# robotics-upo/social_force_window_planner

Measured on AMD Instinct MI355X. Metric: scored trajectories/sec (v x w samples x steps) @ N pedestrians; cmd_vel match, higher is better.
Workload: dtype f64

## Files before the change

include/sfw_hip.h:

```cpp
#ifndef SFW_HIP_H_
#define SFW_HIP_H_

#include <stdint.h>

#ifdef __cplusplus
extern "C" {
#endif

#define SFW_ABI_VERSION 2

typedef enum sfw_status {
  SFW_OK = 0,
  SFW_ERR_INVALID_ARG = -1,
  SFW_ERR_NO_DEVICE = -2,
  SFW_ERR_HIP = -3,
  SFW_ERR_STATE = -4,
  SFW_ERR_UNSUPPORTED = -5
} sfw_status;

#define SFW_COST_INVALID (-1.0)
#define SFW_COST_SKIPPED (-2.0)

#define SFW_ROBOT_ID_NONE INT32_MIN

// ... 109 lines not shown
int sfw_score_samples(sfw_handle h, const sfw_robot_state *rs, const double *vx, const double *vy,
                      const double *vtheta, int32_t n, const sfw_goal_args *args, double *costs_out,
                      sfw_best *best_out);

#define SFW_SEQ_MAX_KNOTS 64
int sfw_sequences_stage(sfw_handle h, const sfw_robot_state *rs, const double *vx, const double *vy,
                        const double *vtheta, int32_t n, int32_t K, const int32_t *knot_step,
                        const sfw_goal_args *args, int64_t index_base);
int sfw_score_sequences(sfw_handle h, const sfw_robot_state *rs, const double *vx, const double *vy,
                        const double *vtheta, int32_t n, int32_t K, const int32_t *knot_step,
                        const sfw_goal_args *args, double *costs_out, sfw_best *best_out);

#define SFW_PERTURB_KEEP_NOMINAL 1
#define SFW_PERTURB_NO_VY        2
#define SFW_PERTURB_KEEP_NORMALS 4
typedef struct sfw_perturb {
  uint64_t seed;
  const double *nominal;
  double sigma[3];
  double lo[3], hi[3];
  int32_t flags, reserved;
} sfw_perturb;
int sfw_sequences_perturb_stage(sfw_handle h, const sfw_robot_state *rs, const sfw_perturb *p, int32_t n, int32_t K,
                                const int32_t *knot_step, const sfw_goal_args *args, int64_t index_base);
int sfw_score_perturbed(sfw_handle h, const sfw_robot_state *rs, const sfw_perturb *p, int32_t n, int32_t K,
                        const int32_t *knot_step, const sfw_goal_args *args, double *costs_out, sfw_best *best_out);
int sfw_sequences_knots(sfw_handle h, int64_t first, int64_t count, double *vx_out, double *vy_out, double *vtheta_out);
int sfw_sequences_normals(sfw_handle h, int64_t first, int64_t count, double *z_out);

#define SFW_ORG_NONE 0
#define SFW_ORG_REGISTER_1 1
#define SFW_ORG_REGISTER_2 2
#define SFW_ORG_FLAT 3
typedef struct sfw_plan_info {
  int32_t split_step;
  int32_t levels;
  int32_t chunks;
  int32_t organisation;
  int64_t classes;
  int64_t class_steps;
  int64_t samples;
  int64_t flat_samples;
  int64_t one_launch;
  int64_t rest_noise_unreproduced;
} sfw_plan_info;
int sfw_grid_plan_info(sfw_handle h, sfw_plan_info *out);
int sfw_plan_shared_prefix(const double *linvels, int32_t nv,
                           const double *angvels, int32_t nw, double vx0,
                           double vtheta0, double acc_x, double acc_theta,
                           double sim_time, int32_t num_steps,
                           int32_t n_agents, int32_t *level_ends,
                           int64_t *level_classes, int32_t cap,
                           int32_t *n_levels);
int sfw_plan_axis_classes(const double *targets, int32_t n, double v0, double a_max, double dt, int32_t max_p,
                          int32_t form, int32_t *counts, int32_t *classes, int32_t *n_levels, int32_t *closed_form);
int sfw_plan_row_blocks(const double *linvels, int32_t nv, const double *angvels, int32_t nw, double vx0,
                        double vtheta0, double acc_x, double acc_theta, double sim_time, int32_t num_steps,
                        int32_t n_agents, int32_t R, int32_t *row0);
#define SFW_K2_AUTO (-1)
#define SFW_K2_REGISTER 0
#define SFW_K2_FLAT 1
int sfw_set_k2_form(sfw_handle h, int32_t form);
int sfw_set_timing(sfw_handle h, int32_t enabled);
int sfw_last_launch_ms(sfw_handle h, int32_t which, float *ms_out);
int sfw_last_clock_ghz(sfw_handle h, double *ghz_out);
int sfw_grid_points(sfw_handle h, int64_t index, double *points_xyth,
                    int32_t points_cap, int32_t *n_points);
int sfw_grid_points_batch(sfw_handle h, int64_t first, int64_t count, double *points_xyth, int32_t *n_points);
int sfw_set_points_capture(sfw_handle h, int32_t enabled);
int sfw_set_footprint_clearance(sfw_handle h, int32_t on);
int sfw_footprint_clearance_info(sfw_handle h, int32_t *built, int32_t *half_width);
int sfw_footprint_clearance_map(sfw_handle h, uint8_t *out, uint64_t cells);
void *sfw_stream(sfw_handle h);

#define SFW_TERM_VEL 0
#define SFW_TERM_DISTANCE 1
#define SFW_TERM_ANGLE 2
#define SFW_TERM_COSTMAP 3
#define SFW_TERM_SOCIAL 4
#define SFW_N_TERMS 5
#define SFW_RESCORE_MAX_K 1024
typedef struct sfw_weights {
  double vel, distance, angle, costmap, social;
} sfw_weights;
int sfw_set_terms_capture(sfw_handle h, int32_t enabled);
int sfw_grid_rescore(sfw_handle h, const sfw_weights *w, int32_t K, sfw_best *best_out, double *costs_out);
int sfw_grid_terms(sfw_handle h, int64_t first, int64_t count, double *terms_out);

#define SFW_BLEND_MAX_L 16
typedef struct sfw_blend_stat {
  double lambda;
  double j_min;
  double eta;
  double sum_w2;
  int64_t n_valid;
  int64_t index_min;
} sfw_blend_stat;
int sfw_grid_blend(sfw_handle h, const double *lambda, int32_t L, const double *bias,
                   sfw_blend_stat *stat_out, double *u_out, double *weights_out);

int sfw_sequences_control_cost(sfw_handle h, double gamma, double *bias_out);
int sfw_grid_blend_control(sfw_handle h, const double *lambda, int32_t L, double gamma, const double *bias,
                           sfw_blend_stat *stat_out, double *u_out, double *weights_out);

#define SFW_MPPI_MAX_ITER 32
typedef struct sfw_mppi {
// ... 158 lines not shown
```

social_force_window_planner_amd/_abi.py:

```python
import ctypes as C

SFW_OK = 0
SFW_ERR_INVALID_ARG = -1
SFW_ERR_NO_DEVICE = -2
SFW_ERR_HIP = -3
SFW_ERR_STATE = -4
SFW_ERR_UNSUPPORTED = -5

SFW_COST_INVALID = -1.0
SFW_COST_SKIPPED = -2.0

SFW_PRECISION_F64 = 0
SFW_PRECISION_F32 = 1
SFW_PRECISION_F64_STRICT = 2

SFW_K2_AUTO, SFW_K2_REGISTER, SFW_K2_FLAT = -1, 0, 1
SFW_ORG_NONE, SFW_ORG_REGISTER_1, SFW_ORG_REGISTER_2, SFW_ORG_FLAT = 0, 1, 2, 3


class SfwParams(C.Structure):
    _fields_ = [
        ("max_vel_x", C.c_double),
        ("sim_time", C.c_double),
        ("sim_granularity", C.c_double),
# ... 82 lines not shown

class SfwBest(C.Structure):
    _fields_ = [
        ("index", C.c_int64),
        ("cost", C.c_double),
        ("vx", C.c_double),
        ("vy", C.c_double),
        ("vtheta", C.c_double),
        ("n_valid", C.c_int64),
    ]

    def as_dict(self):
        return {n: getattr(self, n) for n, _ in self._fields_}


class SfwBestKey(C.Structure):
    _fields_ = [(n, C.c_double) for n in ("cost", "neg_linvel", "abs_angvel", "neg_index")]

    def as_tuple(self):
        return (self.cost, self.neg_linvel, self.abs_angvel, self.neg_index)


class SfwPlanInfo(C.Structure):
    _fields_ = [("split_step", C.c_int32), ("levels", C.c_int32), ("chunks", C.c_int32), ("organisation", C.c_int32),
                ("classes", C.c_int64), ("class_steps", C.c_int64), ("samples", C.c_int64), ("flat_samples", C.c_int64),
                ("one_launch", C.c_int64), ("rest_noise_unreproduced", C.c_int64)]

    def as_dict(self):
        return {"split_step": self.split_step, "levels": self.levels, "chunks": self.chunks, "classes": self.classes,
                "class_steps": self.class_steps, "samples": self.samples, "organisation": self.organisation,
                "flat_samples": self.flat_samples, "one_launch": self.one_launch,
                "rest_noise_unreproduced": self.rest_noise_unreproduced}


EXPORTED_SYMBOLS = (
    "sfw_params_default",
    "sfw_abi_version",
    "sfw_create",
    "sfw_destroy",
    "sfw_set_params",
    "sfw_last_error",
    "sfw_set_costmap",
    "sfw_set_footprint",
    "sfw_set_agents",
    "sfw_score_grid",
    "sfw_score_one",
    "sfw_grid_stage",
    "sfw_grid_launch",
    "sfw_grid_sync",
    "sfw_grid_fetch",
    "sfw_grid_costs_view",
    "sfw_grid_plan_info",
    "sfw_plan_shared_prefix",
    "sfw_plan_row_blocks",
    "sfw_plan_axis_classes",
    "sfw_set_k2_form",
    "sfw_set_timing",
    "sfw_last_launch_ms",
    "sfw_last_clock_ghz",
    "sfw_grid_points",
    "sfw_grid_points_batch",
    "sfw_set_points_capture",
    "sfw_stream",
    "sfw_multi_create",
    "sfw_multi_destroy",
    "sfw_multi_last_error",
    "sfw_multi_describe",
    "sfw_multi_ranks",
    "sfw_multi_rank_handle",
    "sfw_multi_set_params",
    "sfw_multi_set_costmap",
    "sfw_multi_set_footprint",
    "sfw_multi_set_agents",
    "sfw_multi_score_grid",
    "sfw_multi_rank_rows",
    "sfw_multi_last_us",
    "sfw_multi_grid_points",
    "sfw_batch_create",
    "sfw_batch_destroy",
    "sfw_batch_last_error",
    "sfw_batch_size",
    "sfw_batch_member",
    "sfw_batch_launch",
    "sfw_batch_fetch",
    "sfw_batch_score_grid",
    "sfw_batch_describe",
    "sfw_batch_last_us",
    "sfw_batch_set_list_fusion",
    "sfw_batch_get_list_fusion",
    "sfw_batch_score_samples",
    "sfw_batch_score_sequences",
    "sfw_batch_score_perturbed",
    "sfw_ensemble_set_list_fusion",
    "sfw_ensemble_get_list_fusion",
    "sfw_ensemble_batch_desc",
    "sfw_set_terms_capture",
    "sfw_grid_rescore",
    "sfw_grid_terms",
    "sfw_ensemble_create",
    "sfw_ensemble_destroy",
    "sfw_ensemble_last_error",
    "sfw_ensemble_size",
    "sfw_ensemble_member",
    "sfw_ensemble_set_params",
    "sfw_ensemble_set_costmap",
    "sfw_ensemble_set_footprint",
# ... 156 lines not shown
```

social_force_window_planner_amd/csrc/sfw_capi.hip:

```cpp

#include "sfw_device.h"

#include <dlfcn.h>
#include <link.h>

#include <algorithm>
#include <chrono>
#include <cmath>
#include <condition_variable>
#include <functional>
#include <mutex>
#include <thread>
#include <cstdio>
#include <cstdlib>
#include <cstring>
#include <limits>
#include <new>
#include <string>
#include <vector>

namespace {

template <typename T> struct dev_buf {
  T *p = nullptr;
// ... 605 lines not shown
      while (l > 0 && t_at(l - 1) > d) --l;
      lo.push_back(static_cast<int32_t>(l));
      hi.push_back(static_cast<int32_t>(h));
      int32_t classes = (l > 0 ? 1 : 0) + (h < cnt ? 1 : 0);
      if (h > l) classes += run[h - 1] - run[l] + 1;
      n.push_back(classes);
      if (static_cast<size_t>(classes) == cnt) break;
    }
    c.assign(n.size(), std::vector<int32_t>());
    return true;
  }
  void write_level(size_t lv) const {
    const size_t cnt = targets.size();
    const size_t l = static_cast<size_t>(lo[lv]), h = static_cast<size_t>(hi[lv]);
    std::vector<int32_t> &out = c[lv];
    out.resize(cnt);
    const int32_t below = l > 0 ? 1 : 0;
    const int32_t mid = h > l ? run[h - 1] - run[l] + 1 : 0;
    for (size_t k = 0; k < cnt; ++k) {
      int32_t id;
      if (k < l) id = 0;
      else if (k < h) id = below + (run[k] - run[l]);
      else id = below + mid;
      out[static_cast<size_t>(order[k])] = id;
    }
  }
};
bool plan_fast_allowed() {
  static const bool on = [] {
    const char *e = std::getenv("SFW_PLAN_GENERIC");
    return !(e && e[0] == '1');
  }();
  return on;
}
axis_classes classes_of_axis(const std::vector<double> &targets, double v0, double a_max, double dt, int max_p,
                             bool allow_fast = plan_fast_allowed()) {
  axis_classes a;
  a.targets = targets;
  a.v0 = v0;
  a.a_max = a_max;
  a.dt = dt;
  a.max_p = max_p;
  a.build(allow_fast);
  return a;
}
int prefix_max_p(int S) { return std::min(S - 1, 48); }

struct prefix_classes {
  axis_classes rows, own_cols;
  const axis_classes *cols = nullptr;
  int max_p = 0;
  int32_t n_rows_at(int p) const { return rows.n[std::min<size_t>(static_cast<size_t>(p), rows.n.size()) - 1]; }
  int32_t n_cols_at(int p) const { return cols->n[std::min<size_t>(static_cast<size_t>(p), cols->n.size()) - 1]; }
};

void classes_of_grid(prefix_classes &pc, const std::vector<double> &lin, const std::vector<double> &ang, double vx0,
                     double vth0, double acc_x, double acc_theta, double dt, int S, const axis_classes *shared_cols = nullptr) {
  pc.max_p = prefix_max_p(S);
  pc.rows = classes_of_axis(lin, vx0, acc_x, dt, pc.max_p);
  if (shared_cols && shared_cols->made_for(ang, vth0, acc_theta, dt, pc.max_p)) {
    pc.cols = shared_cols;
  } else {
    pc.own_cols = classes_of_axis(ang, vth0, acc_theta, dt, pc.max_p);
    pc.cols = &pc.own_cols;
  }
}

std::vector<int> choose_levels(const prefix_classes &pc, int64_t T, int S, double samples_per_wave, int cus) {
  std::vector<int> steps;
  const double full = step_cost(static_cast<double>(T), samples_per_wave, cus);
  const int last_p = std::min<int>(pc.max_p, static_cast<int>(std::max(pc.rows.n.size(), pc.cols->n.size())));
  std::vector<double> best(static_cast<size_t>(last_p) + 1, 0.0);
  std::vector<int> from(static_cast<size_t>(last_p) + 1, 0);
  double best_total = S * full;
  int best_end = 0;
  for (int p = 1; p <= last_p; ++p) {
    const double c = step_cost(static_cast<double>(pc.n_rows_at(p)) * pc.n_cols_at(p), samples_per_wave, cus);
    const double launch_cost = c < 1.0 ? 0.4 : 1.0;
    best[p] = 1e300;
    for (int q = 0; q < p; ++q) {
      const double v = best[q] + (p - q) * c + launch_cost;
      if (v < best[p]) { best[p] = v; from[p] = q; }
    }
    const double total = best[p] + (S - p) * full;
    if (total < best_total) { best_total = total; best_end = p; }
  }
  if (best_total > 0.97 * S * full) return steps;
  for (int p = best_end; p > 0; p = from[p]) steps.push_back(p);
  std::reverse(steps.begin(), steps.end());
  return steps;
}

void plan_row_blocks(const std::vector<double> &lin, const std::vector<double> &ang, double vx0, double vth0, double acc_x,
                     double acc_theta, double dt, int S, int A, int R, int form, int cus, std::vector<int32_t> &row0) {
  const int64_t nv = static_cast<int64_t>(lin.size()), nw = static_cast<int64_t>(ang.size());
  row0.assign(static_cast<size_t>(R) + 1, 0);
  for (int r = 0; r <= R; ++r) row0[static_cast<size_t>(r)] = static_cast<int32_t>((static_cast<int64_t>(r) * nv) / R);
  if (R <= 1 || A < 2 || S < 2 || (nv / R) * nw < 4096) return;
  prefix_classes pc;
  classes_of_grid(pc, lin, ang, vx0, vth0, acc_x, acc_theta, dt, S);
  const std::vector<int> steps = choose_levels(pc, nv * nw, S, static_cast<double>(sfw_samples_per_wave(A, (nv / R) * nw, form, cus)), cus);
  if (steps.empty()) return;
  std::vector<double> w(static_cast<size_t>(nv), static_cast<double>(nw) * (S - steps.back()));
  int prev = 0;
  for (int p : steps) {
    const std::vector<int32_t> &rc = pc.rows.level(p);
    const double per_class = static_cast<double>(pc.n_cols_at(p)) * (p - prev);
    for (int64_t i = 0; i < nv; ++i)
      if (i == 0 || rc[static_cast<size_t>(i)] != rc[static_cast<size_t>(i - 1)]) w[static_cast<size_t>(i)] += per_class;
    prev = p;
  }
  double total = 0.0;
  for (double v : w) total += v;
  double run = 0.0;
  int r = 1;
  for (int64_t i = 0; i < nv && r < R; ++i) {
    run += w[static_cast<size_t>(i)];
    while (r < R && run >= total * r / R) row0[static_cast<size_t>(r++)] = static_cast<int32_t>(i + 1);
  }
  for (; r < R; ++r) row0[static_cast<size_t>(r)] = static_cast<int32_t>(nv);
}

int plan_prefix(sfw_handle h, int64_t chunk, int S) {
  h->st.prefix_steps.clear();
  h->st.prefix_chunks.clear();
  h->st.cls_ints.clear();
  h->st.cls_max = 0;
  h->st.prefix_class_steps = h->st.prefix_last_classes = 0;
  const int64_t T = static_cast<int64_t>(h->st.nv) * h->st.nw;
  const bool forced = !h->cfg.prefix_env.empty();
  if (h->st.list) return SFW_OK;
  if ((forced && h->cfg.prefix_env[0] == 0) || h->st.A < 2 || S < 2 || h->st.vy_samp != 0.0) return SFW_OK;
  if (!forced && T < 4096) return SFW_OK;
  const int64_t rows_per_chunk = chunk / h->st.nw;
  if (rows_per_chunk < 1) return SFW_OK;
  prefix_classes pc;
  classes_of_grid(pc, h->st.lin, h->st.ang, h->st.rs.vx, h->st.rs.vtheta, h->st.ga.acc_x, h->st.ga.acc_theta, h->live.params.sim_time / S, S,
                  static_cast<const axis_classes *>(h->shared_cols));
  const axis_classes &rc = pc.rows, &cc = *pc.cols;
  const std::vector<int32_t> &nr = pc.rows.n, &nc = pc.cols->n;
  auto level = [](const axis_classes &c, int p) -> const std::vector<int32_t> & { return c.level(p); };
  auto count_at = [](const std::vector<int32_t> &n, int p) { return n[std::min<size_t>(static_cast<size_t>(p), n.size()) - 1]; };
  std::vector<int> steps;
  if (forced) {
    for (int p : h->cfg.prefix_env)
      if (p >= 1 && p <= pc.max_p) steps.push_back(p);
  } else {
    steps = choose_levels(pc, T, S, static_cast<double>(sfw_samples_per_wave(h->st.A, std::min<int64_t>(T, rows_per_chunk * h->st.nw), h->live.k2_form, h->cfg.n_cu)), h->cfg.n_cu);
  }
  if (steps.empty()) return SFW_OK;
  const size_t n_lv = steps.size();

  std::vector<int32_t> ints;
  ints.swap(h->st.cls_ints);
  ints.clear();
  ints.reserve(static_cast<size_t>(2 * n_lv + 2) * static_cast<size_t>(h->st.nv + h->st.nw));
  auto append = [&](const std::vector<int32_t> &v) {
    const size_t o = ints.size();
    ints.insert(ints.end(), v.begin(), v.end());
    return o;
  };
  std::vector<int32_t> ids;
  auto relabel = [&ids](const std::vector<int32_t> &cls, int64_t i0, int64_t i1, std::vector<int32_t> &local,
                        std::vector<int32_t> &rep) {
    ids.assign(cls.size(), -1);
    local.clear();
    rep.clear();
    local.reserve(static_cast<size_t>(i1 - i0));
    rep.reserve(static_cast<size_t>(i1 - i0));
    for (int64_t i = i0; i < i1; ++i) {
      int32_t &id = ids[static_cast<size_t>(cls[static_cast<size_t>(i)])];
      if (id < 0) {
        id = static_cast<int32_t>(rep.size());
        rep.push_back(static_cast<int32_t>(i - i0));
      }
      local.push_back(id);
    }
  };
  struct axis_level { std::vector<int32_t> local, rep, src; };
  auto axis_levels = [&](const axis_classes &cls, int64_t i0, int64_t i1) {
    std::vector<axis_level> out(n_lv);
    for (size_t l = 0; l < n_lv; ++l) {
      relabel(level(cls, steps[l]), i0, i1, out[l].local, out[l].rep);
      if (l > 0) {
        out[l].src.reserve(out[l].rep.size());
        for (int32_t r : out[l].rep) out[l].src.push_back(out[l - 1].local[static_cast<size_t>(r)]);
      }
    }
    return out;
  };
  const std::vector<axis_level> cols = axis_levels(cc, 0, h->st.nw);
  std::vector<size_t> o_col_rep(n_lv), o_col_src(n_lv);
  for (size_t l = 0; l < n_lv; ++l) {
    o_col_rep[l] = append(cols[l].rep);
    o_col_src[l] = append(cols[l].src);
  }
  h->st.prefix_o_col_cls = append(cols[n_lv - 1].local);
  int64_t max_cls = 0;
  for (int64_t r0 = 0; r0 < h->st.nv; r0 += rows_per_chunk) {
    const int64_t r1 = std::min<int64_t>(h->st.nv, r0 + rows_per_chunk);
    const std::vector<axis_level> rows = axis_levels(rc, r0, r1);
    chunk_plan cp;
    for (size_t l = 0; l < n_lv; ++l) {
      level_tables t;
      t.n_row = static_cast<int32_t>(rows[l].rep.size());
      t.n_col = static_cast<int32_t>(cols[l].rep.size());
      t.o_row_rep = append(rows[l].rep);
      t.o_row_src = append(rows[l].src);
      t.o_col_rep = o_col_rep[l];
      t.o_col_src = o_col_src[l];
      cp.lv.push_back(t);
      const int64_t n = static_cast<int64_t>(t.n_row) * t.n_col;
      max_cls = std::max(max_cls, n);
      h->st.prefix_class_steps += n * (steps[l] - (l ? steps[l - 1] : 0));
      if (l + 1 == n_lv) h->st.prefix_last_classes += n;
    }
    cp.o_row_cls = append(rows[n_lv - 1].local);
    h->st.prefix_chunks.push_back(cp);
  }
  h->st.cls_ints.swap(ints);
  h->st.cls_max = max_cls;
  h->st.cls_two = n_lv > 1;
  if (std::getenv("SFW_DEBUG_PLAN")) {
    std::fprintf(stderr, "[sfw] shared prefix, %d x %d samples, S=%d, %zu chunk(s):", h->st.nv, h->st.nw, S, h->st.prefix_chunks.size());
    for (size_t l = 0; l < n_lv; ++l)
      std::fprintf(stderr, " [%d,%d) %d x %d;", l ? steps[l - 1] : 0, steps[l], count_at(nr, steps[l]), count_at(nc, steps[l]));
    std::fprintf(stderr, " [%d,%d) samples\n", steps.back(), S);
  }
  h->st.prefix_steps = steps;
  h->st.prefix_S = S;
  h->st.prefix_chunk = rows_per_chunk * h->st.nw;
  return SFW_OK;
}

void rest_forces(const sfw_params &p, const std::vector<std::pair<int32_t, int32_t>> &pairs, const double *pos, const double *vel,
                 int A, double *out) {
  for (int i = 0; i < 2 * A; ++i) out[i] = 0.0;
  for (const auto &pr : pairs) {
    const int i = pr.first, j = pr.second;
    const double dx = pos[2 * j] - pos[2 * i], dy = pos[2 * j + 1] - pos[2 * i + 1];
    const double dn = std::sqrt(dx * dx + dy * dy);
    if (!(dn > 0.0)) continue;
    const double ux = dx / dn, uy = dy / dn;
    const double wx = vel[2 * i] - vel[2 * j], wy = vel[2 * i + 1] - vel[2 * j + 1];
    const double ix = p.sfm_lambda * wx + ux, iy = p.sfm_lambda * wy + uy;
    const double il = std::sqrt(ix * ix + iy * iy);
    if (!(il > 0.0)) continue;
    const double ex = ix / il, ey = iy / il;
    double theta = std::atan2(uy, ux) - std::atan2(ey, ex);
    while (theta <= -M_PI) theta += 2.0 * M_PI;
    while (theta > M_PI) theta -= 2.0 * M_PI;
    const double B = p.sfm_gamma * il;
    if (theta != 0.0) {
      const double sq = p.sfm_n * B * theta;
      const double fa = -(theta > 0.0 ? 1.0 : -1.0) * std::exp(-dn / B - sq * sq);
      out[2 * i] += p.sfm_force_factor_social * fa * -ey;
      out[2 * i + 1] += p.sfm_force_factor_social * fa * ex;
    }
  }
}

bool pinned_rest_table(const sfw_params &p, const sfw_robot_state &rs, const double *pos, const sfw_agent_const *cst, int A,
                       double *out) {
  bool any = false;
  for (int i = 1; i < A; ++i) any |= (cst[i].desired_velocity == 0.0);
  if (!any) return false;
  out[0] = rs.x;
  out[1] = rs.y;
  out[2] = out[3] = 0.0;
  for (int i = 0; i < A; ++i) out[4 + i] = 0.0;
  auto pair_at_rest = [&](double mx, double my, double ox, double oy, double &fx, double &fy, double &lx, double &ly) {
    fx = fy = lx = ly = 0.0;
    const double dx = ox - mx, dy = oy - my;
    const double dn = std::sqrt(dx * dx + dy * dy);
    if (!(dn > 0.0)) return;
    const double ux = dx / dn, uy = dy / dn;
    const double ix = p.sfm_lambda * 0.0 + ux, iy = p.sfm_lambda * 0.0 + uy;
    const double il = std::sqrt(ix * ix + iy * iy);
    if (!(il > 0.0)) return;
// ... 1609 lines not shown
  const size_t rows = 3 * static_cast<size_t>(h->st.nk), row = sizeof(double) * static_cast<size_t>(count);
  SFW_HIP(h, hipSetDevice(h->device));
  if (rows * row > h->pin_knots.cap) SFW_HIP(h, hipStreamSynchronize(h->stream));
  SFW_HIP(h, h->pin_knots.reserve(rows * row));
  SFW_HIP(h, hipMemcpy2DAsync(h->pin_knots.p, row, h->normals.p + first, sizeof(double) * static_cast<size_t>(n), row, rows,
                              hipMemcpyDeviceToHost, h->stream));
  SFW_HIP(h, wait_stream(h));
  std::memcpy(z_out, h->pin_knots.p, rows * row);
  return SFW_OK;
}

int sfw_score_one(sfw_handle h, const sfw_robot_state *rs, double vx_samp, double vy_samp, double vtheta_samp,
                  const sfw_goal_args *args, double *cost_out, double *points_xyth, int32_t points_cap,
                  int32_t *n_points) {
  if (!h) return SFW_ERR_INVALID_ARG;
  if (!cost_out) return fail(h, SFW_ERR_INVALID_ARG, "score_one: cost_out is NULL");
  if (int e = stage_one(h, rs, args, vx_samp, vy_samp, vtheta_samp)) return e;
  consume_stage consumed{h};
  const int S = num_steps_of(h->live.params);
  const size_t head = kOneHead, pts_bytes = sizeof(double) * 3 * static_cast<size_t>(S);
  sfw_launch L;
  fill_launch(h, L, 0, 1, 1);
  L.force_alive = (points_xyth && points_cap > 0) || n_points ? 1 : 0;
  {
    sfw_launch C = L;
    C.sel_out = nullptr;
    C.cycle_counter = nullptr;
    if (sfw_cycle_applies(C)) {
      if (head + pts_bytes > h->pin_one.cap) SFW_HIP(h, hipStreamSynchronize(h->stream));
      SFW_HIP(h, h->pin_one.reserve(head + pts_bytes));
      score_one_outputs_at(C, h->pin_one.p);
      arena_by_kernel(h, C);
      SFW_HIP(h, launch_cycle_of(C, h->stream));
      SFW_HIP(h, arena_fetched(h));
      SFW_HIP(h, wait_stream(h));
      score_one_unpack(h->pin_one.p, cost_out, points_xyth, points_cap, n_points);
      return SFW_OK;
    }
    if (int e = flush_arena(h)) return e;
  }
  SFW_HIP(h, h->one_out.reserve(head + pts_bytes));
  score_one_outputs_at(L, h->one_out.p);
  SFW_HIP(h, sfw_launch_rollout(L, h->stream));
  SFW_HIP(h, launch_social_of(L, h->stream));
  if (L.path_on) SFW_HIP(h, sfw_launch_path_add(L.costs, L.path_p, h->st.path_weight, 0, 1, h->stream));
  const size_t fetch = head + ((points_xyth && points_cap > 0) ? pts_bytes : 0);
  SFW_HIP(h, h->pin_out.reserve(fetch));
  SFW_HIP(h, hipMemcpyAsync(h->pin_out.p, h->one_out.p, fetch, hipMemcpyDeviceToHost, h->stream));
  SFW_HIP(h, hipStreamSynchronize(h->stream));
  score_one_unpack(h->pin_out.p, cost_out, points_xyth, points_cap, n_points);
  return SFW_OK;
}

int sfw_plan_shared_prefix(const double *linvels, int32_t nv, const double *angvels, int32_t nw, double vx0, double vtheta0,
                           double acc_x, double acc_theta, double sim_time, int32_t num_steps, int32_t n_agents,
                           int32_t *level_ends, int64_t *level_classes, int32_t cap, int32_t *n_levels) {
  if (!linvels || !angvels || nv <= 0 || nw <= 0 || num_steps < 1 || !n_levels || cap < 0 ||
      (cap > 0 && (!level_ends || !level_classes)))
    return SFW_ERR_INVALID_ARG;
  *n_levels = 0;
  const int64_t T = static_cast<int64_t>(nv) * nw;
  if (n_agents < 2 || num_steps < 2 || T < 4096) return SFW_OK;
  const std::vector<double> lin(linvels, linvels + nv), ang(angvels, angvels + nw);
  prefix_classes pc;
  classes_of_grid(pc, lin, ang, vx0, vtheta0, acc_x, acc_theta, sim_time / num_steps, num_steps);
  const int cus = env_device_cus(SFW_DEFAULT_CUS);
  const std::vector<int> steps = choose_levels(pc, T, num_steps, static_cast<double>(sfw_samples_per_wave(n_agents, T, SFW_K2_AUTO, cus)), cus);
  *n_levels = static_cast<int32_t>(steps.size());
  for (size_t l = 0; l < steps.size() && l < static_cast<size_t>(cap); ++l) {
    level_ends[l] = steps[l];
    level_classes[l] = static_cast<int64_t>(pc.n_rows_at(steps[l])) * pc.n_cols_at(steps[l]);
  }
  return SFW_OK;
}

int sfw_plan_axis_classes(const double *targets, int32_t n, double v0, double a_max, double dt, int32_t max_p, int32_t form,
                          int32_t *counts, int32_t *classes, int32_t *n_levels, int32_t *closed_form) {
  if (!targets || n <= 0 || max_p < 1 || !counts || !n_levels || (form != 0 && form != 1)) return SFW_ERR_INVALID_ARG;
  if (!all_finite(targets, static_cast<size_t>(n)) || !std::isfinite(v0) || !std::isfinite(a_max) || !std::isfinite(dt))
    return SFW_ERR_INVALID_ARG;
  const axis_classes a = classes_of_axis(std::vector<double>(targets, targets + n), v0, a_max, dt, max_p, form == 0);
  *n_levels = static_cast<int32_t>(a.n.size());
  if (closed_form) *closed_form = a.fast ? 1 : 0;
  for (size_t l = 0; l < a.n.size(); ++l) {
    counts[l] = a.n[l];
    if (classes) std::memcpy(classes + l * static_cast<size_t>(n), a.level(static_cast<int>(l) + 1).data(), sizeof(int32_t) * static_cast<size_t>(n));
  }
  return SFW_OK;
}

int sfw_plan_row_blocks(const double *linvels, int32_t nv, const double *angvels, int32_t nw, double vx0, double vtheta0,
                        double acc_x, double acc_theta, double sim_time, int32_t num_steps, int32_t n_agents, int32_t R,
                        int32_t *row0) {
  if (!linvels || !angvels || nv <= 0 || nw <= 0 || num_steps < 1 || R < 1 || !row0) return SFW_ERR_INVALID_ARG;
  if (!all_finite(linvels, static_cast<size_t>(nv)) || !all_finite(angvels, static_cast<size_t>(nw))) return SFW_ERR_INVALID_ARG;
  const std::vector<double> lin(linvels, linvels + nv), ang(angvels, angvels + nw);
  std::vector<int32_t> cuts;
  plan_row_blocks(lin, ang, vx0, vtheta0, acc_x, acc_theta, sim_time / num_steps, num_steps, n_agents, R, SFW_K2_AUTO,
                  env_device_cus(SFW_DEFAULT_CUS), cuts);
  std::memcpy(row0, cuts.data(), sizeof(int32_t) * (static_cast<size_t>(R) + 1));
  return SFW_OK;
}

int sfw_grid_plan_info(sfw_handle h, sfw_plan_info *out) {
  if (!h || !out) return SFW_ERR_INVALID_ARG;
  if (!h->st.valid) return fail(h, SFW_ERR_STATE, "grid_plan_info before grid_stage");
  const int64_t T = static_cast<int64_t>(h->st.nv) * h->st.nw;
  out->split_step = h->st.prefix_steps.empty() ? 0 : h->st.prefix_steps.back();
  out->levels = static_cast<int32_t>(h->st.prefix_steps.size());
  out->samples = T;
  out->classes = h->st.prefix_last_classes;
  out->class_steps = h->st.prefix_class_steps;
  if (!h->st.prefix_steps.empty()) {
    out->chunks = static_cast<int32_t>(h->st.prefix_chunks.size());
  } else {
    int64_t chunk = h->st.table_chunk;
    if (chunk > T) chunk = T;
    out->chunks = chunk > 0 ? static_cast<int32_t>((T + chunk - 1) / chunk) : 0;
  }
  out->organisation = sfw_social_organisation(h->st.A, out->chunks > 0 ? (T + out->chunks - 1) / out->chunks : T, h->st.O, h->live.k2_form, h->cfg.n_cu);
  out->flat_samples = sfw_social_flat_items(h->st.A, h->st.O, h->st.NG, out->chunks > 0 ? (T + out->chunks - 1) / out->chunks : T, h->live.k2_form, h->cfg.n_cu);
  out->rest_noise_unreproduced = rest_noise_unreproduced(h) ? 1 : 0;
  out->one_launch = 0;
  if (out->chunks == 1 && h->st.prefix_steps.empty()) {
    sfw_launch L;
    fill_launch(h, L, 0, T, T);
// ... 1885 lines not shown
```

social_force_window_planner_amd/planner.py:

```python
from __future__ import annotations

import ctypes as C
import os
import subprocess

import numpy as np

from ._abi import (
    EXPORTED_SYMBOLS,
    SFW_ENSEMBLE_MAX,
    SFW_ENSEMBLE_MEAN,
    SFW_ERR_NO_DEVICE,
    SFW_OK,
    SfwAgent,
    SfwBatchDesc,
    SfwBest,
    SfwBestKey,
    SfwBlendStat,
    SFW_BLEND_MAX_L,
    SfwGoalArgs,
    SfwMppi,
    SFW_MPPI_MAX_ITER,
    SfwParams,
    SfwPerturb,
# ... 43 lines not shown
        L.sfw_params_default.argtypes = [C.POINTER(SfwParams)]
        L.sfw_params_default.restype = None
        L.sfw_abi_version.restype = C.c_int
        L.sfw_create.argtypes = [C.POINTER(SfwParams), C.c_int, C.POINTER(vp)]
        L.sfw_destroy.argtypes = [vp]
        L.sfw_set_params.argtypes = [vp, C.POINTER(SfwParams)]
        L.sfw_last_error.argtypes = [vp]
        L.sfw_last_error.restype = C.c_char_p
        L.sfw_set_costmap.argtypes = [vp, vp, C.c_uint32, C.c_uint32, C.c_double, C.c_double, C.c_double]
        L.sfw_set_footprint.argtypes = [vp, vp, C.c_int32]
        L.sfw_set_agents.argtypes = [vp, vp, C.c_int32, vp, C.c_int32]
        L.sfw_score_grid.argtypes = [vp, C.POINTER(SfwRobotState), vp, C.c_int32, vp, C.c_int32,
                                     C.POINTER(SfwGoalArgs), vp, C.POINTER(SfwBest)]
        L.sfw_score_one.argtypes = [vp, C.POINTER(SfwRobotState), C.c_double, C.c_double, C.c_double,
                                    C.POINTER(SfwGoalArgs), C.POINTER(C.c_double), vp, C.c_int32,
                                    C.POINTER(C.c_int32)]
        L.sfw_grid_stage.argtypes = [vp, C.POINTER(SfwRobotState), vp, C.c_int32, vp, C.c_int32,
                                     C.POINTER(SfwGoalArgs), C.c_int64]
        L.sfw_grid_launch.argtypes = [vp]
        L.sfw_grid_sync.argtypes = [vp]
        L.sfw_grid_fetch.argtypes = [vp, vp, C.POINTER(SfwBest), C.POINTER(SfwBestKey)]
        L.sfw_grid_plan_info.argtypes = [vp, C.POINTER(SfwPlanInfo)]
        L.sfw_set_k2_form.argtypes = [vp, C.c_int32]
        L.sfw_set_timing.argtypes = [vp, C.c_int32]
        L.sfw_last_launch_ms.argtypes = [vp, C.c_int32, C.POINTER(C.c_float)]
        L.sfw_last_clock_ghz.argtypes = [vp, C.POINTER(C.c_double)]
        L.sfw_grid_points.argtypes = [vp, C.c_int64, vp, C.c_int32, C.POINTER(C.c_int32)]
        L.sfw_grid_points_batch.argtypes = [vp, C.c_int64, C.c_int64, vp, vp]
        L.sfw_set_points_capture.argtypes = [vp, C.c_int32]
        L.sfw_stream.argtypes = [vp]
        L.sfw_stream.restype = vp
        L.sfw_multi_create.argtypes = [C.POINTER(SfwParams), C.POINTER(C.c_int), C.c_int32, C.c_int32, C.POINTER(vp)]
        L.sfw_multi_destroy.argtypes = [vp]
        L.sfw_multi_last_error.argtypes = [vp]
        L.sfw_multi_last_error.restype = C.c_char_p
        L.sfw_multi_ranks.argtypes = [vp]
        L.sfw_multi_ranks.restype = C.c_int32
        L.sfw_multi_rank_handle.argtypes = [vp, C.c_int32]
        L.sfw_multi_rank_handle.restype = vp
        L.sfw_multi_set_params.argtypes = [vp, C.POINTER(SfwParams)]
        L.sfw_multi_set_costmap.argtypes = [vp, vp, C.c_uint32, C.c_uint32, C.c_double, C.c_double, C.c_double]
        L.sfw_multi_set_footprint.argtypes = [vp, vp, C.c_int32]
        L.sfw_multi_set_agents.argtypes = [vp, vp, C.c_int32, vp, C.c_int32]
        L.sfw_multi_score_grid.argtypes = [vp, C.POINTER(SfwRobotState), vp, C.c_int32, vp, C.c_int32,
                                           C.POINTER(SfwGoalArgs), vp, C.POINTER(SfwBest)]
        L.sfw_multi_last_us.argtypes = [vp, C.c_int32, C.POINTER(C.c_double)]
        L.sfw_multi_rank_rows.argtypes = [vp, C.c_int32, C.POINTER(C.c_int32), C.POINTER(C.c_int32)]
        L.sfw_plan_row_blocks.argtypes = [vp, C.c_int32, vp, C.c_int32, C.c_double, C.c_double, C.c_double, C.c_double,
                                          C.c_double, C.c_int32, C.c_int32, C.c_int32, vp]
        L.sfw_grid_costs_view.argtypes = [vp]
        L.sfw_grid_costs_view.restype = C.c_void_p
        L.sfw_plan_shared_prefix.argtypes = [vp, C.c_int32, vp, C.c_int32, C.c_double, C.c_double, C.c_double, C.c_double,
                                             C.c_double, C.c_int32, C.c_int32, vp, vp, C.c_int32, C.POINTER(C.c_int32)]
        L.sfw_multi_grid_points.argtypes = [vp, C.c_int64, vp, C.c_int32, C.POINTER(C.c_int32)]
        L.sfw_batch_create.argtypes = [C.POINTER(SfwParams), C.c_int, C.c_int32, C.POINTER(vp)]
        L.sfw_batch_destroy.argtypes = [vp]
        L.sfw_batch_last_error.argtypes = [vp]
        L.sfw_batch_last_error.restype = C.c_char_p
        L.sfw_batch_size.argtypes = [vp]
        L.sfw_batch_size.restype = C.c_int32
        L.sfw_batch_member.argtypes = [vp, C.c_int32]
        L.sfw_batch_member.restype = vp
        L.sfw_batch_launch.argtypes = [vp]
        L.sfw_batch_fetch.argtypes = [vp, vp]
        L.sfw_batch_score_grid.argtypes = [vp, vp, vp, C.c_int32, vp, C.c_int32, vp, vp]
        L.sfw_batch_describe.argtypes = [vp, C.POINTER(SfwBatchDesc)]
        L.sfw_batch_last_us.argtypes = [vp, C.c_int32, C.POINTER(C.c_double)]
        L.sfw_set_terms_capture.argtypes = [vp, C.c_int32]
        L.sfw_grid_rescore.argtypes = [vp, C.POINTER(SfwWeights), C.c_int32, C.POINTER(SfwBest), vp]
        L.sfw_grid_terms.argtypes = [vp, C.c_int64, C.c_int64, vp]
        L.sfw_ensemble_create.argtypes = [C.POINTER(SfwParams), C.c_int, C.c_int32, C.POINTER(vp)]
        L.sfw_ensemble_destroy.argtypes = [vp]
        L.sfw_ensemble_last_error.argtypes = [vp]
        L.sfw_ensemble_last_error.restype = C.c_char_p
        L.sfw_ensemble_size.argtypes = [vp]
        L.sfw_ensemble_size.restype = C.c_int32
        L.sfw_ensemble_member.argtypes = [vp, C.c_int32]
        L.sfw_ensemble_member.restype = vp
        L.sfw_ensemble_set_params.argtypes = [vp, C.POINTER(SfwParams)]
        L.sfw_ensemble_set_costmap.argtypes = [vp, vp, C.c_uint32, C.c_uint32, C.c_double, C.c_double, C.c_double]
        L.sfw_ensemble_set_footprint.argtypes = [vp, vp, C.c_int32]
        L.sfw_ensemble_set_hypothesis.argtypes = [vp, C.c_int32, vp, C.c_int32, vp, C.c_int32]
        L.sfw_ensemble_score_grid.argtypes = [vp, C.POINTER(SfwRobotState), vp, C.c_int32, vp, C.c_int32,
                                              C.POINTER(SfwGoalArgs), C.c_int32, vp, vp, vp, C.POINTER(SfwBest)]
        L.sfw_ensemble_aggregate.argtypes = [vp, C.c_int32, vp, vp, vp, C.POINTER(SfwBest)]
        L.sfw_ensemble_last_us.argtypes = [vp, C.c_int32, C.POINTER(C.c_double)]
        L.sfw_samples_stage.argtypes = [vp, C.POINTER(SfwRobotState), vp, vp, vp, C.c_int32, C.POINTER(SfwGoalArgs), C.c_int64]
        L.sfw_score_samples.argtypes = [vp, C.POINTER(SfwRobotState), vp, vp, vp, C.c_int32, C.POINTER(SfwGoalArgs), vp,
                                        C.POINTER(SfwBest)]
        L.sfw_score_one_crowd.argtypes = [vp, C.POINTER(SfwRobotState), C.c_double, C.c_double, C.c_double,
                                          C.POINTER(SfwGoalArgs), C.POINTER(C.c_double), vp, vp, vp, C.c_int32, C.c_int32,
                                          C.POINTER(C.c_int32)]
        L.sfw_grid_crowd.argtypes = [vp, C.c_int64, C.POINTER(C.c_double), vp, vp, vp, C.c_int32, C.c_int32,
                                     C.POINTER(C.c_int32)]
        L.sfw_sequences_stage.argtypes = [vp, C.POINTER(SfwRobotState), vp, vp, vp, C.c_int32, C.c_int32, vp,
                                          C.POINTER(SfwGoalArgs), C.c_int64]
        L.sfw_score_sequences.argtypes = [vp, C.POINTER(SfwRobotState), vp, vp, vp, C.c_int32, C.c_int32, vp,
                                          C.POINTER(SfwGoalArgs), vp, C.POINTER(SfwBest)]
        L.sfw_grid_blend.argtypes = [vp, vp, C.c_int32, vp, C.POINTER(SfwBlendStat), vp, vp]
        L.sfw_sequences_perturb_stage.argtypes = [vp, C.POINTER(SfwRobotState), C.POINTER(SfwPerturb), C.c_int32, C.c_int32, vp,
                                                  C.POINTER(SfwGoalArgs), C.c_int64]
        L.sfw_score_perturbed.argtypes = [vp, C.POINTER(SfwRobotState), C.POINTER(SfwPerturb), C.c_int32, C.c_int32, vp,
                                          C.POINTER(SfwGoalArgs), vp, C.POINTER(SfwBest)]
        L.sfw_sequences_knots.argtypes = [vp, C.c_int64, C.c_int64, vp, vp, vp]
        L.sfw_sequences_normals.argtypes = [vp, C.c_int64, C.c_int64, vp]
        L.sfw_ensemble_score_sequences.argtypes = [vp, C.POINTER(SfwRobotState), vp, vp, vp, C.c_int32, C.c_int32, vp,
# ... 493 lines not shown
        if count is None:
            nv, nw = self._grid if self._grid is not None else (0, 0)
            count = max(nv * nw - first, 0)
        out = np.empty((count, SFW_N_TERMS), dtype=np.float64)
        self._check(lib().sfw_grid_terms(self._h, first, count, out.ctypes.data), "sfw_grid_terms")
        return out

    def rescore(self, weights, want_costs=False):
        w = np.ascontiguousarray(np.asarray(weights, dtype=np.float64).reshape(-1, SFW_N_TERMS))
        K = w.shape[0]
        best = (SfwBest * max(K, 1))()
        costs = None
        if want_costs and self._grid is not None:
            nv, nw = self._grid
            costs = np.empty((K, nv * nw), dtype=np.float64)
        self._check(lib().sfw_grid_rescore(self._h, C.cast(w.ctypes.data, C.POINTER(SfwWeights)), K, best,
                                           costs.ctypes.data if costs is not None else None), "sfw_grid_rescore")
        return [best[k].as_dict() for k in range(K)], costs

    def blend(self, lambdas, bias=None, want_weights=False, gamma=None):
        nv, nw = self._grid if self._grid is not None else (0, 0)
        K = getattr(self, "_n_knots", 1) if self._grid is not None else 64
        return _blend(self._check, lib().sfw_grid_blend, lib().sfw_grid_blend_control, self._h, nv * nw, K, lambdas, bias,
                      want_weights, gamma)

    def control_cost(self, gamma):
        n = self._grid[0] if self._grid is not None else 0
        out = np.zeros(max(n, 1), dtype=np.float64)
        self._check(lib().sfw_sequences_control_cost(self._h, float(gamma), out.ctypes.data), "sfw_sequences_control_cost")
        return out[:n]

    def mppi_run(self, robot_state, n, seed, nominal, sigma, lo, hi, knot_steps, goal_args, iterations, lam, gamma, flags=0):
        head, tail, K, I, stats, plans, _alive = _mppi_args(robot_state, n, seed, nominal, sigma, lo, hi, knot_steps, goal_args,
                                                            iterations, lam, gamma, flags)
        best = SfwBest()
        self._check(lib().sfw_mppi_run(self._h, *head, *tail, C.byref(best)), "sfw_mppi_run")
        self._mark_staged((n, 1), knots=K)
        return [stats[i].as_dict() for i in range(I)], plans, best.as_dict()


def plan_row_blocks(linvels, angvels, robot_state, goal_args, sim_time, num_steps, n_agents, n_ranks):
    lin, ang = _f64(linvels), _f64(angvels)
    row0 = np.zeros(n_ranks + 1, dtype=np.int32)
    rc = lib().sfw_plan_row_blocks(lin.ctypes.data, len(lin), ang.ctypes.data, len(ang), robot_state[3], robot_state[5],
                                   goal_args[0], goal_args[2], sim_time, num_steps, n_agents, n_ranks, row0.ctypes.data)
    if rc != SFW_OK:
        raise SfwError(rc, "sfw_plan_row_blocks")
    return row0


def planned_share(linvels, angvels, robot_state, goal_args, sim_time, num_steps, n_agents):
    lin, ang = _f64(linvels), _f64(angvels)
    ends, cls, n = np.zeros(64, dtype=np.int32), np.zeros(64, dtype=np.int64), C.c_int32()
    rc = lib().sfw_plan_shared_prefix(lin.ctypes.data, len(lin), ang.ctypes.data, len(ang), robot_state[3], robot_state[5],
                                      goal_args[0], goal_args[2], sim_time, num_steps, n_agents, ends.ctypes.data,
                                      cls.ctypes.data, 64, C.byref(n))
    if rc != SFW_OK:
        raise SfwError(rc, "sfw_plan_shared_prefix")
    k = min(n.value, 64)
    if k == 0:
        return 1.0
    total = len(lin) * len(ang) * num_steps
    prev, class_steps = 0, 0
    for l in range(k):
        class_steps += int(cls[l]) * int(ends[l] - prev)
        prev = int(ends[l])
    return (class_steps + len(lin) * len(ang) * (num_steps - prev)) / total


def plan_info_of_rank(multi, r):
    info = SfwPlanInfo()
    h = lib().sfw_multi_rank_handle(multi._m, r)
    rc = lib().sfw_grid_plan_info(h, C.byref(info))
    if rc != SFW_OK:
        raise SfwError(rc, "sfw_grid_plan_info")
    return info.as_dict()


class PreparedGrid:

    def __init__(self, scorer, robot_state, linvels, angvels, goal_args, index_base, zero_copy=False):
        self.scorer = scorer
        self.lin, self.ang = _f64(linvels).copy(), _f64(angvels).copy()
        self.rs, self.ga = SfwRobotState(*robot_state), SfwGoalArgs(*goal_args)
        self.costs = np.empty(len(self.lin) * len(self.ang), dtype=np.float64)
        self.best, self.key = SfwBest(), SfwBestKey()
        L = lib()
        self._stage, self._launch, self._fetch = L.sfw_grid_stage, L.sfw_grid_launch, L.sfw_grid_fetch
        self._stage_args = (scorer._h, C.byref(self.rs), self.lin.ctypes.data, len(self.lin), self.ang.ctypes.data, len(self.ang),
                            C.byref(self.ga), index_base)
        self._fetch_args = (scorer._h, self.costs.ctypes.data, C.byref(self.best), C.byref(self.key))
        self._fetch_args_nocost = (scorer._h, None, C.byref(self.best), C.byref(self.key))
        scorer._mark_staged((len(self.lin), len(self.ang)))
        self.zero_copy = zero_copy
        self._view, self._view_ptr, self._view_arr = L.sfw_grid_costs_view, None, None

    def step(self, want_costs=True):
        s = self.scorer
        rc = self._stage(*self._stage_args)
        if rc != SFW_OK:
            s._check(rc, "sfw_grid_stage")
        rc = self._launch(s._h)
        if rc != SFW_OK:
            s._check(rc, "sfw_grid_launch")
        if want_costs and self.zero_copy:
            rc = self._fetch(*self._fetch_args_nocost)
            if rc != SFW_OK:
                s._check(rc, "sfw_grid_fetch")
            p = self._view(s._h)
            if p:
                if p != self._view_ptr:
# ... 413 lines not shown
```

Before: 7.828 million.

## Share prefix levels by lagged angular classes to shrink per-level work items

Changes the shared-prefix planner so that the angular class at step p is taken from level p-1 (one column for p<2). The reasoning is that the angular state at step p depends only on commands applied up to p-1, so more samples can share a prefix item. This lowers the number of distinct items per level and lets the level chooser pick longer shared prefixes, cutting redundant simulation steps. It relies on that lagged-equivalence assumption holding for every cost term, and it adds an items-based planning entry point in C and Python.

```diff
diff --git a/include/sfw_hip.h b/include/sfw_hip.h
--- a/include/sfw_hip.h
+++ b/include/sfw_hip.h
@@ -185,6 +185,9 @@
                            int32_t n_agents, int32_t *level_ends,
                            int64_t *level_classes, int32_t cap,
                            int32_t *n_levels);
+int sfw_plan_shared_prefix_items(const double *linvels, int32_t nv, const double *angvels, int32_t nw, double vx0,
+                                 double vtheta0, double acc_x, double acc_theta, double sim_time, int32_t num_steps,
+                                 int32_t n_agents, int32_t *level_ends, int64_t *level_items, int32_t cap, int32_t *n_levels);
 int sfw_plan_axis_classes(const double *targets, int32_t n, double v0, double a_max, double dt, int32_t max_p,
                           int32_t form, int32_t *counts, int32_t *classes, int32_t *n_levels, int32_t *closed_form);
 int sfw_plan_row_blocks(const double *linvels, int32_t nv, const double *angvels, int32_t nw, double vx0,
diff --git a/social_force_window_planner_amd/_abi.py b/social_force_window_planner_amd/_abi.py
--- a/social_force_window_planner_amd/_abi.py
+++ b/social_force_window_planner_amd/_abi.py
@@ -158,6 +158,7 @@
     "sfw_grid_costs_view",
     "sfw_grid_plan_info",
     "sfw_plan_shared_prefix",
+    "sfw_plan_shared_prefix_items",
     "sfw_plan_row_blocks",
     "sfw_plan_axis_classes",
     "sfw_set_k2_form",
diff --git a/social_force_window_planner_amd/csrc/sfw_capi.hip b/social_force_window_planner_amd/csrc/sfw_capi.hip
--- a/social_force_window_planner_amd/csrc/sfw_capi.hip
+++ b/social_force_window_planner_amd/csrc/sfw_capi.hip
@@ -681,6 +681,10 @@
   int max_p = 0;
   int32_t n_rows_at(int p) const { return rows.n[std::min<size_t>(static_cast<size_t>(p), rows.n.size()) - 1]; }
   int32_t n_cols_at(int p) const { return cols->n[std::min<size_t>(static_cast<size_t>(p), cols->n.size()) - 1]; }
+  int32_t n_item_cols_at(int p) const { return p >= 2 ? n_cols_at(p - 1) : 1; }
+  const std::vector<int32_t> &item_cols(int p) const { return p >= 2 ? cols->level(p - 1) : one_col; }
+  int64_t n_items_at(int p) const { return static_cast<int64_t>(n_rows_at(p)) * n_item_cols_at(p); }
+  std::vector<int32_t> one_col;
 };
 
 void classes_of_grid(prefix_classes &pc, const std::vector<double> &lin, const std::vector<double> &ang, double vx0,
@@ -693,18 +697,19 @@
     pc.own_cols = classes_of_axis(ang, vth0, acc_theta, dt, pc.max_p);
     pc.cols = &pc.own_cols;
   }
+  pc.one_col.assign(ang.size(), 0);
 }
 
 std::vector<int> choose_levels(const prefix_classes &pc, int64_t T, int S, double samples_per_wave, int cus) {
   std::vector<int> steps;
   const double full = step_cost(static_cast<double>(T), samples_per_wave, cus);
-  const int last_p = std::min<int>(pc.max_p, static_cast<int>(std::max(pc.rows.n.size(), pc.cols->n.size())));
+  const int last_p = std::min<int>(pc.max_p, static_cast<int>(std::max(pc.rows.n.size(), pc.cols->n.size() + 1)));
   std::vector<double> best(static_cast<size_t>(last_p) + 1, 0.0);
   std::vector<int> from(static_cast<size_t>(last_p) + 1, 0);
   double best_total = S * full;
   int best_end = 0;
   for (int p = 1; p <= last_p; ++p) {
-    const double c = step_cost(static_cast<double>(pc.n_rows_at(p)) * pc.n_cols_at(p), samples_per_wave, cus);
+    const double c = step_cost(static_cast<double>(pc.n_items_at(p)), samples_per_wave, cus);
     const double launch_cost = c < 1.0 ? 0.4 : 1.0;
     best[p] = 1e300;
     for (int q = 0; q < p; ++q) {
@@ -734,7 +739,7 @@
   int prev = 0;
   for (int p : steps) {
     const std::vector<int32_t> &rc = pc.rows.level(p);
-    const double per_class = static_cast<double>(pc.n_cols_at(p)) * (p - prev);
+    const double per_class = static_cast<double>(pc.n_item_cols_at(p)) * (p - prev);
     for (int64_t i = 0; i < nv; ++i)
       if (i == 0 || rc[static_cast<size_t>(i)] != rc[static_cast<size_t>(i - 1)]) w[static_cast<size_t>(i)] += per_class;
     prev = p;
@@ -766,8 +771,8 @@
   prefix_classes pc;
   classes_of_grid(pc, h->st.lin, h->st.ang, h->st.rs.vx, h->st.rs.vtheta, h->st.ga.acc_x, h->st.ga.acc_theta, h->live.params.sim_time / S, S,
                   static_cast<const axis_classes *>(h->shared_cols));
-  const axis_classes &rc = pc.rows, &cc = *pc.cols;
-  const std::vector<int32_t> &nr = pc.rows.n, &nc = pc.cols->n;
+  const axis_classes &rc = pc.rows;
+  const std::vector<int32_t> &nr = pc.rows.n;
   auto level = [](const axis_classes &c, int p) -> const std::vector<int32_t> & { return c.level(p); };
   auto count_at = [](const std::vector<int32_t> &n, int p) { return n[std::min<size_t>(static_cast<size_t>(p), n.size()) - 1]; };
   std::vector<int> steps;
@@ -807,10 +812,10 @@
     }
   };
   struct axis_level { std::vector<int32_t> local, rep, src; };
-  auto axis_levels = [&](const axis_classes &cls, int64_t i0, int64_t i1) {
+  auto axis_levels = [&](const axis_classes *cls, int64_t i0, int64_t i1) {
     std::vector<axis_level> out(n_lv);
     for (size_t l = 0; l < n_lv; ++l) {
-      relabel(level(cls, steps[l]), i0, i1, out[l].local, out[l].rep);
+      relabel(cls ? level(*cls, steps[l]) : pc.item_cols(steps[l]), i0, i1, out[l].local, out[l].rep);
       if (l > 0) {
         out[l].src.reserve(out[l].rep.size());
         for (int32_t r : out[l].rep) out[l].src.push_back(out[l - 1].local[static_cast<size_t>(r)]);
@@ -818,7 +823,7 @@
     }
     return out;
   };
-  const std::vector<axis_level> cols = axis_levels(cc, 0, h->st.nw);
+  const std::vector<axis_level> cols = axis_levels(nullptr, 0, h->st.nw);
   std::vector<size_t> o_col_rep(n_lv), o_col_src(n_lv);
   for (size_t l = 0; l < n_lv; ++l) {
     o_col_rep[l] = append(cols[l].rep);
@@ -828,7 +833,7 @@
   int64_t max_cls = 0;
   for (int64_t r0 = 0; r0 < h->st.nv; r0 += rows_per_chunk) {
     const int64_t r1 = std::min<int64_t>(h->st.nv, r0 + rows_per_chunk);
-    const std::vector<axis_level> rows = axis_levels(rc, r0, r1);
+    const std::vector<axis_level> rows = axis_levels(&rc, r0, r1);
     chunk_plan cp;
     for (size_t l = 0; l < n_lv; ++l) {
       level_tables t;
@@ -853,7 +858,7 @@
   if (std::getenv("SFW_DEBUG_PLAN")) {
     std::fprintf(stderr, "[sfw] shared prefix, %d x %d samples, S=%d, %zu chunk(s):", h->st.nv, h->st.nw, S, h->st.prefix_chunks.size());
     for (size_t l = 0; l < n_lv; ++l)
-      std::fprintf(stderr, " [%d,%d) %d x %d;", l ? steps[l - 1] : 0, steps[l], count_at(nr, steps[l]), count_at(nc, steps[l]));
+      std::fprintf(stderr, " [%d,%d) %d x %d;", l ? steps[l - 1] : 0, steps[l], count_at(nr, steps[l]), pc.n_item_cols_at(steps[l]));
     std::fprintf(stderr, " [%d,%d) samples\n", steps.back(), S);
   }
   h->st.prefix_steps = steps;
@@ -2569,9 +2574,9 @@
   return SFW_OK;
 }
 
-int sfw_plan_shared_prefix(const double *linvels, int32_t nv, const double *angvels, int32_t nw, double vx0, double vtheta0,
-                           double acc_x, double acc_theta, double sim_time, int32_t num_steps, int32_t n_agents,
-                           int32_t *level_ends, int64_t *level_classes, int32_t cap, int32_t *n_levels) {
+static int plan_shared_prefix(const double *linvels, int32_t nv, const double *angvels, int32_t nw, double vx0, double vtheta0,
+                              double acc_x, double acc_theta, double sim_time, int32_t num_steps, int32_t n_agents,
+                              int32_t *level_ends, int64_t *level_classes, int32_t cap, int32_t *n_levels, bool items) {
   if (!linvels || !angvels || nv <= 0 || nw <= 0 || num_steps < 1 || !n_levels || cap < 0 ||
       (cap > 0 && (!level_ends || !level_classes)))
     return SFW_ERR_INVALID_ARG;
@@ -2586,9 +2591,21 @@
   *n_levels = static_cast<int32_t>(steps.size());
   for (size_t l = 0; l < steps.size() && l < static_cast<size_t>(cap); ++l) {
     level_ends[l] = steps[l];
-    level_classes[l] = static_cast<int64_t>(pc.n_rows_at(steps[l])) * pc.n_cols_at(steps[l]);
-  }
-  return SFW_OK;
+    level_classes[l] = items ? pc.n_items_at(steps[l]) : static_cast<int64_t>(pc.n_rows_at(steps[l])) * pc.n_cols_at(steps[l]);
+  }
+  return SFW_OK;
+}
+int sfw_plan_shared_prefix(const double *linvels, int32_t nv, const double *angvels, int32_t nw, double vx0, double vtheta0,
+                           double acc_x, double acc_theta, double sim_time, int32_t num_steps, int32_t n_agents,
+                           int32_t *level_ends, int64_t *level_classes, int32_t cap, int32_t *n_levels) {
+  return plan_shared_prefix(linvels, nv, angvels, nw, vx0, vtheta0, acc_x, acc_theta, sim_time, num_steps, n_agents, level_ends,
+                            level_classes, cap, n_levels, false);
+}
+int sfw_plan_shared_prefix_items(const double *linvels, int32_t nv, const double *angvels, int32_t nw, double vx0, double vtheta0,
+                                 double acc_x, double acc_theta, double sim_time, int32_t num_steps, int32_t n_agents,
+                                 int32_t *level_ends, int64_t *level_items, int32_t cap, int32_t *n_levels) {
+  return plan_shared_prefix(linvels, nv, angvels, nw, vx0, vtheta0, acc_x, acc_theta, sim_time, num_steps, n_agents, level_ends,
+                            level_items, cap, n_levels, true);
 }
 
 int sfw_plan_axis_classes(const double *targets, int32_t n, double v0, double a_max, double dt, int32_t max_p, int32_t form,
diff --git a/social_force_window_planner_amd/planner.py b/social_force_window_planner_amd/planner.py
--- a/social_force_window_planner_amd/planner.py
+++ b/social_force_window_planner_amd/planner.py
@@ -119,6 +119,7 @@
         L.sfw_grid_costs_view.restype = C.c_void_p
         L.sfw_plan_shared_prefix.argtypes = [vp, C.c_int32, vp, C.c_int32, C.c_double, C.c_double, C.c_double, C.c_double,
                                              C.c_double, C.c_int32, C.c_int32, vp, vp, C.c_int32, C.POINTER(C.c_int32)]
+        L.sfw_plan_shared_prefix_items.argtypes = L.sfw_plan_shared_prefix.argtypes
         L.sfw_multi_grid_points.argtypes = [vp, C.c_int64, vp, C.c_int32, C.POINTER(C.c_int32)]
         L.sfw_batch_create.argtypes = [C.POINTER(SfwParams), C.c_int, C.c_int32, C.POINTER(vp)]
         L.sfw_batch_destroy.argtypes = [vp]
@@ -718,11 +719,11 @@
 def planned_share(linvels, angvels, robot_state, goal_args, sim_time, num_steps, n_agents):
     lin, ang = _f64(linvels), _f64(angvels)
     ends, cls, n = np.zeros(64, dtype=np.int32), np.zeros(64, dtype=np.int64), C.c_int32()
-    rc = lib().sfw_plan_shared_prefix(lin.ctypes.data, len(lin), ang.ctypes.data, len(ang), robot_state[3], robot_state[5],
-                                      goal_args[0], goal_args[2], sim_time, num_steps, n_agents, ends.ctypes.data,
-                                      cls.ctypes.data, 64, C.byref(n))
+    rc = lib().sfw_plan_shared_prefix_items(lin.ctypes.data, len(lin), ang.ctypes.data, len(ang), robot_state[3], robot_state[5],
+                                            goal_args[0], goal_args[2], sim_time, num_steps, n_agents, ends.ctypes.data,
+                                            cls.ctypes.data, 64, C.byref(n))
     if rc != SFW_OK:
-        raise SfwError(rc, "sfw_plan_shared_prefix")
+        raise SfwError(rc, "sfw_plan_shared_prefix_items")
     k = min(n.value, 64)
     if k == 0:
         return 1.0
```

After: 7.994 million (median of 6 runs). +2.1%, better.
